# Arthur151/ROMP

Measured on NVIDIA H100. Metric: frames/sec 512x512 ROMP-HRNet32 (whole hot path), higher is better.
Workload: dtype bf16

## Files before the change

romp_b200/csrc/conv_block_tc.cu:

```cuda
#include "conv_tc.cuh"
#include "tc_device.cuh"

namespace b200romp {

namespace {

constexpr int kBlkThreads = 384;
constexpr int kRowB = 128;
constexpr int kHaloH = 20;
constexpr int kTapBytes = 64 * kRowB;
constexpr int kHalfTapBytes = 64 * 64;

template <bool FOLD>
struct BlkCfg {
  static constexpr int kWBytes = FOLD ? 3 * (kTapBytes + 2 * kHalfTapBytes) : 9 * kTapBytes;
  static constexpr int kTW = FOLD ? 16 : 8;
  static constexpr int kHaloW = kTW + 4;
  static constexpr int kN1 = FOLD ? 192 : 128;
  static constexpr int kN2 = 8 * kTW;
  static constexpr int kG2 = kN2 / 8;
  static constexpr int kMidRows = 2 * kN1;
  static constexpr int kStagePayload = kHaloH * kHaloW * kRowB;
  static constexpr int kStageBytes = ((kMidRows + 2 * kHaloW + 2) * kRowB + 1023) / 1024 * 1024;
  static constexpr int kMidBytes = kMidRows * kRowB;
// ... 22 lines not shown
}

__device__ __forceinline__ void consumers_bar_sync() { asm volatile("bar.sync 1, 256;" ::: "memory"); }

__device__ __forceinline__ void ldmatrix_x4_trans(uint32_t (&r)[4], uint32_t addr) {
  asm volatile("ldmatrix.sync.aligned.m8n8.x4.trans.shared.b16 {%0, %1, %2, %3}, [%4];"
               : "=r"(r[0]), "=r"(r[1]), "=r"(r[2]), "=r"(r[3])
               : "r"(addr));
}
__device__ __forceinline__ void stmatrix_x4_trans(uint32_t addr, const uint32_t (&r)[4]) {
  asm volatile("stmatrix.sync.aligned.m8n8.x4.trans.shared.b16 [%0], {%1, %2, %3, %4};" ::"r"(addr), "r"(r[0]), "r"(r[1]), "r"(r[2]),
               "r"(r[3])
               : "memory");
}
__device__ __forceinline__ void st_shared_zero16(uint32_t addr) {
  asm volatile("st.shared.v4.b32 [%0], {%1, %1, %1, %1};" ::"r"(addr), "r"(0) : "memory");
}
template <int N>
__device__ __forceinline__ void wgmma_bf16(float (&d)[N / 2], uint64_t a, uint64_t b, uint32_t scale_d) {
  if constexpr (N == 192) wgmma_n192_bf16(d, a, b, scale_d);
  else if constexpr (N == 128) wgmma_n128_bf16(d, a, b, scale_d);
  else wgmma_n64(d, a, b, scale_d, false);
}
template <typename T>
__device__ __forceinline__ T opaque(T v) {
  uint64_t u = (uint64_t)v;
  asm volatile("mov.b64 %0, %0;" : "+l"(u));
  return (T)u;
}
__device__ __forceinline__ uint32_t pack_bf16x2(float a, float b) {
  const __nv_bfloat162 v = __floats2bfloat162_rn(a, b);
  return *reinterpret_cast<const uint32_t*>(&v);
}

struct BlkThread {
  int g, w, l;
};
template <bool FOLD>
__device__ __forceinline__ int c2_oy0(int g) { return FOLD ? 0 : 8 * g; }
template <bool FOLD>
__device__ __forceinline__ int c2_ox0(int g) { return FOLD ? 8 * g : 0; }
struct BlkTile {
  int n, y0, x0;
  __device__ BlkTile(int tile, int tiles_x, int per_frame, int tw) {
    n = tile / per_frame;
    const int rem = tile % per_frame;
    y0 = (rem / tiles_x) * 16;
    x0 = (rem % tiles_x) * tw;
  }
};

template <bool FOLD>
__device__ __forceinline__ void conv1_issue(float (&acc)[BlkCfg<FOLD>::kN1 / 2], uint32_t a_base, uint32_t w1_base, int row0) {
  constexpr int kHaloW = BlkCfg<FOLD>::kHaloW, kN1 = BlkCfg<FOLD>::kN1;
#pragma unroll
  for (int j = 0; j < kN1 / 2; ++j) acc[j] = 0.f;
  uint32_t scale_d = 0;
  wgmma_fence();
#pragma unroll
  for (int tap = 0; tap < 9; ++tap) {
    const uint32_t b_tap = a_base + (uint32_t)((row0 + (tap / 3) * kHaloW + tap % 3) * kRowB);
#pragma unroll
    for (int k = 0; k < 4; ++k) {
      if (blk_skip<FOLD>(tap, k)) continue;
      wgmma_bf16<kN1>(acc, w_desc<FOLD>(w1_base, tap, k), make_smem_desc(b_tap + k * 32, 8 * kRowB, kSw128), scale_d);
      scale_d = 1;
    }
  }
  wgmma_commit();
}

template <bool FOLD>
__device__ __forceinline__ void load_residual(uint32_t (&rv)[BlkCfg<FOLD>::kG2][2], uint32_t a_base, const BlkThread& th) {
  constexpr int kHaloW = BlkCfg<FOLD>::kHaloW;
  const int q = th.l >> 3;
#pragma unroll
  for (int j0 = 0; j0 < BlkCfg<FOLD>::kG2; j0 += 2) {
    const int hr = (c2_oy0<FOLD>(th.g) + j0 + (q >> 1) + 2) * kHaloW + c2_ox0<FOLD>(th.g) + (th.l & 7) + 2;
    uint32_t r[4];
    ldmatrix_x4_trans(r, a_base + hr * kRowB + (((2 * th.w + (q & 1)) ^ (hr & 7)) << 4));
    rv[j0][0] = r[0]; rv[j0][1] = r[1]; rv[j0 + 1][0] = r[2]; rv[j0 + 1][1] = r[3];
  }
}

template <bool FOLD>
__device__ __forceinline__ void mid_epilogue(const float (&acc)[BlkCfg<FOLD>::kN1 / 2], uint32_t mid_base, const float* b1p, const ConvParams& p,
                                             const BlkTile& tl, const BlkThread& th, int row0) {
  constexpr int kHaloW = BlkCfg<FOLD>::kHaloW, kTW = BlkCfg<FOLD>::kTW, kN1 = BlkCfg<FOLD>::kN1;
  const float bias[2] = {__ldg(b1p + 16 * th.w + (th.l >> 2)), __ldg(b1p + 16 * th.w + (th.l >> 2) + 8)};
  const int q = th.l >> 3;
#pragma unroll
  for (int j0 = 0; j0 < kN1 / 8; j0 += 2) {
    uint32_t r[4];
#pragma unroll
    for (int i = 0; i < 4; ++i) {
      const int j = j0 + (i >> 1), e = i & 1;
      r[i] = pack_bf16x2(fmaxf(acc[4 * j + 2 * e] + bias[e], 0.f), fmaxf(acc[4 * j + 2 * e + 1] + bias[e], 0.f));
    }
    const int m = row0 + 8 * (j0 + (q >> 1)) + (th.l & 7);
    stmatrix_x4_trans(mid_base + m * kRowB + (((2 * th.w + (q & 1)) ^ (m & 7)) << 4), r);
  }
  if (tl.y0 > 0 && tl.x0 > 0 && tl.y0 + 16 < p.Hout && tl.x0 + kTW < p.Wout) return;
  __syncwarp();
  constexpr int kRingRow = kTW + 2, kRing = 2 * kRingRow + 2 * 18;
#pragma unroll 1
  for (int i = th.l; i < 2 * kRing; i += 32) {
    const int k = i >> 1;
    const int my = k < 2 * kRingRow ? (k < kRingRow ? 0 : 17) : (k - 2 * kRingRow) % 18;
    const int mx = k < 2 * kRingRow ? k % kRingRow : (k - 2 * kRingRow < 18 ? 0 : kTW + 1);
    const int m = my * kHaloW + mx;
    if (m >= row0 && m < row0 + kN1 && ((unsigned)(tl.y0 - 1 + my) >= (unsigned)p.Hout || (unsigned)(tl.x0 - 1 + mx) >= (unsigned)p.Wout))
      st_shared_zero16(mid_base + m * kRowB + (((2 * th.w + (i & 1)) ^ (m & 7)) << 4));
  }
}

template <bool FOLD>
__device__ __forceinline__ void conv2_issue(float (&acc2)[BlkCfg<FOLD>::kN2 / 2], uint32_t mid_base, uint32_t w2_base, int g) {
  constexpr int kHaloW = BlkCfg<FOLD>::kHaloW, kN2 = BlkCfg<FOLD>::kN2;
#pragma unroll
  for (int j = 0; j < kN2 / 2; ++j) acc2[j] = 0.f;
  uint32_t scale_d = 0;
  wgmma_fence();
#pragma unroll
  for (int tap = 0; tap < 9; ++tap) {
    const uint32_t b_tap = mid_base + (uint32_t)(((c2_oy0<FOLD>(g) + tap / 3) * kHaloW + c2_ox0<FOLD>(g) + tap % 3) * kRowB);
#pragma unroll
    for (int k = 0; k < 4; ++k) {
      if (blk_skip<FOLD>(tap, k)) continue;
      wgmma_bf16<kN2>(acc2, w_desc<FOLD>(w2_base, tap, k), make_smem_desc(b_tap + k * 32, kHaloW * kRowB, kSw128), scale_d);
      scale_d = 1;
    }
  }
  wgmma_commit();
}

template <bool FOLD>
__device__ __forceinline__ void out_epilogue(const float (&acc2)[BlkCfg<FOLD>::kN2 / 2], const uint32_t (&rv)[BlkCfg<FOLD>::kG2][2],
                                             const float* b2p, const ConvParams& p, const BlkTile& tl, const BlkThread& th) {
  __nv_bfloat16* out = reinterpret_cast<__nv_bfloat16*>(p.out);
  const int c = 16 * th.w + (th.l >> 2);
  const float bias[2] = {__ldg(b2p + c), __ldg(b2p + c + 8)};
  const int odd = (th.l >> 2) & 1;
  const int x = tl.x0 + c2_ox0<FOLD>(th.g) + 2 * (th.l & 3) + odd;
#pragma unroll
  for (int j = 0; j < BlkCfg<FOLD>::kG2; ++j) {
    uint16_t h[2][2];
#pragma unroll
    for (int e = 0; e < 2; ++e) {
      const float2 r = res_pair(rv[j][e]);
      const float a = (acc2[4 * j + 2 * e] + bias[e]) + r.x, b = (acc2[4 * j + 2 * e + 1] + bias[e]) + r.y;
      h[e][0] = __bfloat16_as_ushort(__float2bfloat16_rn(fmaxf(a, 0.f)));
      h[e][1] = __bfloat16_as_ushort(__float2bfloat16_rn(fmaxf(b, 0.f)));
    }
    const uint32_t send = odd ? (uint32_t)h[0][0] | ((uint32_t)h[1][0] << 16) : (uint32_t)h[0][1] | ((uint32_t)h[1][1] << 16);
    const uint32_t recv = __shfl_xor_sync(0xffffffffu, send, 4);
    const size_t pix = ((size_t)tl.n * p.Hout + tl.y0 + c2_oy0<FOLD>(th.g) + j) * p.Wout + x;
    uint32_t* o = reinterpret_cast<uint32_t*>(out + pix * p.out_C + p.out_c_off + (c & ~1));
#pragma unroll
    for (int e = 0; e < 2; ++e) {
      const uint32_t theirs = (recv >> (16 * e)) & 0xFFFFu;
      o[4 * e] = odd ? (theirs | ((uint32_t)h[e][1] << 16)) : ((uint32_t)h[e][0] | (theirs << 16));
    }
  }
}

}

template <bool FOLD>
__global__ void __launch_bounds__(kBlkThreads, 1)
conv_block_tc_kernel(const __grid_constant__ CUtensorMap tmap, const ConvParams p, const uint8_t* __restrict__ w1pack,
                     const uint8_t* __restrict__ w2pack, const float* __restrict__ bias1, int tiles_x, int tiles_y, int num_tiles) {
  using Cfg = BlkCfg<FOLD>;
  constexpr int kWBytes = Cfg::kWBytes, kStageBytes = Cfg::kStageBytes;
  extern __shared__ uint8_t smem_raw[];
  uint8_t* smem = reinterpret_cast<uint8_t*>((reinterpret_cast<uintptr_t>(smem_raw) + 1023) & ~(uintptr_t)1023);
  uint8_t* sW1 = smem;
  uint8_t* sW2 = smem + kWBytes;
  uint8_t* sA = smem + 2 * kWBytes;
  uint8_t* sMid = sA + kStageBytes;
  uint64_t* full = reinterpret_cast<uint64_t*>(sMid + Cfg::kMidBytes);
  uint64_t* empty = full + 1;
  uint64_t* w_full = full + 2;

  const int warp = threadIdx.x >> 5;
  if (threadIdx.x == 0) {
    mbar_init(full, 1);
    mbar_init(empty, 256);
    mbar_init(w_full, 1);
    fence_barrier_init();
  }
  __syncthreads();
  pdl_trigger();
  const int per_frame = tiles_x * tiles_y;

  if (warp == 0) {
    if (elect_one()) {
      mbar_arrive_expect_tx(w_full, 2 * kWBytes);
      for (int off = 0; off < kWBytes; off += kTapBytes) {
        bulk_copy_g2s(sW1 + off, w1pack + off, kTapBytes, w_full);
        bulk_copy_g2s(sW2 + off, w2pack + off, kTapBytes, w_full);
      }
      pdl_wait();
      const uint64_t pol = l2_policy_stream();
      uint32_t phase = 0;
      for (int tile = blockIdx.x; tile < num_tiles; tile += gridDim.x, phase ^= 1) {
        const BlkTile tl(tile, tiles_x, per_frame, Cfg::kTW);
        mbar_wait(empty, phase ^ 1);
        mbar_arrive_expect_tx(full, Cfg::kStagePayload);
        tma_load_4d(sA, &tmap, full, 0, tl.x0 - 2, tl.y0 - 2, tl.n, pol);
      }
    }
  } else if (warp >= 4) {
    const int t = threadIdx.x & 127;
    const BlkThread th{(warp >> 2) - 1, t >> 5, t & 31};
    pdl_wait();
    mbar_wait(w_full, 0);
    float acc[Cfg::kN1 / 2], acc2[Cfg::kN2 / 2];
    uint32_t rv[Cfg::kG2][2];
    const int row0 = th.g * Cfg::kN1;
    uint32_t phase = 0;
    for (int tile = blockIdx.x; tile < num_tiles; tile += gridDim.x, phase ^= 1) {
      const uint32_t w1_base = opaque(smem_u32(sW1)), w2_base = opaque(smem_u32(sW2)), a_base = opaque(smem_u32(sA)),
                     mid_base = opaque(smem_u32(sMid));
      const float* b1p = opaque(bias1);
      const float* b2p = opaque(p.bias);
      const BlkTile tl(tile, tiles_x, per_frame, Cfg::kTW);
      mbar_wait(full, phase);
      conv1_issue<FOLD>(acc, a_base, w1_base, row0);
      load_residual<FOLD>(rv, a_base, th);
      wgmma_wait<0>();
      mbar_arrive(empty);
      consumers_bar_sync();
      mid_epilogue<FOLD>(acc, mid_base, b1p, p, tl, th, row0);
      fence_proxy_async();
      consumers_bar_sync();
      conv2_issue<FOLD>(acc2, mid_base, w2_base, th.g);
      wgmma_wait<0>();
      out_epilogue<FOLD>(acc2, rv, b2p, p, tl, th);
    }
  }
}

bool tc_block_supported(const ConvParams& p, bool fold) {
  if (p.in_dtype != B200ROMP_BF16 || p.out_dtype != B200ROMP_BF16 || p.res_dtype != B200ROMP_BF16) return false;
  if (p.cin != 64 || p.cout != 64 || p.up != 1 || p.out_nchw || p.pow_channel >= 0 || p.input_norm || !p.relu) return false;
  if (p.Hin != p.Hout || p.Win != p.Wout || p.Hout % 16 != 0 || p.Wout % (fold ? BlkCfg<true>::kTW : BlkCfg<false>::kTW) != 0) return false;
  if (p.in_C % 8 != 0 || p.in_c_off % 8 != 0 || p.out_C % 8 != 0 || p.out_c_off % 8 != 0) return false;
  if (p.res != p.in || p.res_C != p.in_C || p.res_c_off != p.in_c_off || p.res_broadcast) return false;
  return (reinterpret_cast<uintptr_t>(p.in) & 15) == 0;
}

static int block_pack_weights(const float* w_oihw, bool fold, void** d_out, std::vector<void*>* allocs) {
  if (!fold) return tc_pack_weights(w_oihw, 64, 64, 9, 64, d_out, allocs, kRowB, 2);
  const std::vector<uint8_t> full = tc_pack_image(w_oihw, 64, 64, 9, 64, kRowB, 2);
  const std::vector<uint8_t> half = tc_pack_image(w_oihw, 64, 64, 9, 64, 64, 2);
  std::vector<uint8_t> img(BlkCfg<true>::kWBytes);
  for (int tap = 0; tap < 9; ++tap) {
    uint8_t* dst = img.data() + w_tap_off(true, tap);
    if (tap % 3 == 1) memcpy(dst, full.data() + (size_t)tap * kTapBytes, kTapBytes);
    else memcpy(dst, half.data() + (size_t)(2 * tap + (tap % 3 == 0 ? 1 : 0)) * kHalfTapBytes, kHalfTapBytes);
  }
  *d_out = upload(img.data(), img.size(), allocs);
  return *d_out ? B200ROMP_OK : B200ROMP_ECUDA;
}

int tc_block_prepare(const ConvParams& p, const float* w1_oihw, const float* b1, const float* w2_oihw, int sm_count,
                     TcConvPlan* plan, std::vector<void*>* allocs) {
  plan->kind = 60;
  plan->eb = 2;
  plan->cin = plan->cout = plan->nt = 64;
  plan->grid_x = sm_count;
  plan->grid_y = 1;
  plan->stages = 1;
  plan->smem_bytes = plan->fold ? BlkCfg<true>::kSmemBytes : BlkCfg<false>::kSmemBytes;
  int rc = block_pack_weights(w1_oihw, plan->fold, &plan->d_wpack, allocs);
  if (rc) return rc;
  rc = block_pack_weights(w2_oihw, plan->fold, &plan->d_wpack2, allocs);
  if (rc) return rc;
  plan->d_bias1 = static_cast<const float*>(upload(b1, 64 * sizeof(float), allocs));
  if (!plan->d_bias1) return B200ROMP_ECUDA;
  rc = tc_encode_nhwc_input(&plan->tmap_in, p, 2, 64, plan->fold ? BlkCfg<true>::kHaloW : BlkCfg<false>::kHaloW, kHaloH,
                            CU_TENSOR_MAP_SWIZZLE_128B, "conv_block_tc");
  if (rc) return rc;
  B2R_CUDA_OK(cudaFuncSetAttribute(conv_block_tc_kernel<false>, cudaFuncAttributeMaxDynamicSharedMemorySize, BlkCfg<false>::kSmemBytes));
  B2R_CUDA_OK(cudaFuncSetAttribute(conv_block_tc_kernel<true>, cudaFuncAttributeMaxDynamicSharedMemorySize, BlkCfg<true>::kSmemBytes));
  return B200ROMP_OK;
}

int tc_block_launch(const TcConvPlan& plan, const ConvParams& p, cudaStream_t stream) {
  const int tiles_x = p.Wout / (plan.fold ? BlkCfg<true>::kTW : BlkCfg<false>::kTW), tiles_y = p.Hout / 16;
  const int num_tiles = tiles_x * tiles_y * p.B;
  const dim3 grid(std::min(plan.grid_x, num_tiles));
  auto kern = plan.fold ? conv_block_tc_kernel<true> : conv_block_tc_kernel<false>;
  B2R_CUDA_OK(tc_launch(kern, grid, kBlkThreads, plan.smem_bytes, stream, plan.tmap_in, p, reinterpret_cast<const uint8_t*>(plan.d_wpack),
                        reinterpret_cast<const uint8_t*>(plan.d_wpack2), plan.d_bias1, tiles_x, tiles_y, num_tiles));
  return B200ROMP_OK;
}

}
```

romp_b200/csrc/conv_tc.cu:

```cuda
#include <mutex>

#include "conv_tc.cuh"
#include "tc_device.cuh"

namespace b200romp {

thread_local int g_tc_pdl_override = -1;

constexpr int kTcThreads = 384;
constexpr int kMaxRings = 2;

__host__ __device__ constexpr int s2_row_bytes(int cin, int eb) { return cin * eb >= 512 ? 64 : (cin * eb < 128 ? cin * eb : 128); }

__host__ __device__ constexpr int tc_num_rings(int stages) { return stages >= 4 ? kMaxRings : 1; }
__host__ __device__ constexpr int tc_ring_size(int stages, int ring) { return tc_num_rings(stages) == 1 ? stages : (stages + 1 - ring) / 2; }
__host__ __device__ constexpr int tc_ring_base(int stages, int ring) { return ring ? (stages + 1) / 2 : 0; }

template <int MODE, int CIN, int NT, int EB>
struct TcCfg {
  static constexpr bool S2 = MODE == 2;
  static constexpr int KS = MODE == 1 ? 1 : 3;
  static constexpr int TAPS = KS * KS;
  static constexpr int PAD = KS / 2;
  static constexpr int ROWB = S2 ? s2_row_bytes(CIN, EB) : tc_row_bytes(KS, CIN, EB);
  static constexpr int CW = ROWB / EB;
  static constexpr int KCH = CIN / CW;
  static constexpr int KSTEPS = ROWB / 32;
  static constexpr uint32_t LAYOUT = tc_layout(ROWB);
  static constexpr int HW_ = 8 + 2 * PAD;
  static constexpr int HH = 16 + 2 * PAD;
  __host__ __device__ static constexpr int BH(int i) { return i < 2 ? 17 : 16; }
  __host__ __device__ static constexpr int BW(int i) { return (i & 1) ? 8 : 9; }
  __host__ __device__ static constexpr int SUB_BYTES(int i) { return (BH(i) * BW(i) * ROWB + 1023) / 1024 * 1024; }
  __host__ __device__ static constexpr int SUB_OFF(int i) { return i == 0 ? 0 : SUB_OFF(i - 1) + SUB_BYTES(i - 1); }
  static constexpr int STAGE_PAYLOAD = S2 ? (17 * 9 + 17 * 8 + 16 * 9 + 16 * 8) * ROWB : HH * HW_ * ROWB;
  static constexpr int STAGE_BYTES = S2 ? SUB_OFF(3) + SUB_BYTES(3) : (STAGE_PAYLOAD + 1023) / 1024 * 1024;
  static constexpr int BTILE = NT * ROWB;
  static constexpr int B_BYTES = TAPS * KCH * BTILE;
  static constexpr bool FOLDABLE = MODE == 3 && CIN == 64 && NT == 64 && EB == 2;
};

template <int MODE, int CIN, int NT, int EB, bool GENERIC>
__global__ void __launch_bounds__(kTcThreads, 1)
conv_tc_kernel(const __grid_constant__ CUtensorMap tmap, const __grid_constant__ S2Maps s2maps, const ConvParams p,
               const uint8_t* __restrict__ wpack, int tiles_x, int tiles_y, int num_tiles, int stages, unsigned kmask) {
  using Cfg = TcCfg<MODE, CIN, NT, EB>;
  extern __shared__ uint8_t smem_raw[];
  uint8_t* smem = reinterpret_cast<uint8_t*>((reinterpret_cast<uintptr_t>(smem_raw) + 1023) & ~(uintptr_t)1023);
  uint8_t* sB = smem;
  uint8_t* sA = smem + Cfg::B_BYTES;
  uint64_t* full = reinterpret_cast<uint64_t*>(sA + (size_t)stages * Cfg::STAGE_BYTES);
  uint64_t* empty = full + stages;
  uint64_t* b_full = empty + stages;

  const int warp = threadIdx.x >> 5;
  if (threadIdx.x == 0) {
    for (int i = 0; i < stages; ++i) {
      mbar_init(&full[i], 1);
      mbar_init(&empty[i], 4);
    }
    mbar_init(b_full, 1);
    fence_barrier_init();
  }
  __syncthreads();
  pdl_trigger();
  const int per_frame = tiles_x * tiles_y;
  const int nrings = tc_num_rings(stages);

  if (warp == 0) {
    if (elect_one()) {
      mbar_arrive_expect_tx(b_full, Cfg::B_BYTES);
      const uint8_t* wsrc = wpack + (size_t)blockIdx.y * Cfg::B_BYTES;
      for (int i = 0; i < Cfg::TAPS * Cfg::KCH; ++i)
        bulk_copy_g2s(sB + (size_t)i * Cfg::BTILE, wsrc + (size_t)i * Cfg::BTILE, Cfg::BTILE, b_full);
      pdl_wait();
      const uint64_t pol = l2_policy_stream();
      int stage = 0, stage_other = 0;
      uint32_t phase = 0, phase_other = 0;
      int it = 0;
      for (int tile = blockIdx.x; tile < num_tiles; tile += gridDim.x, ++it) {
        const int n = tile / per_frame, rem = tile % per_frame;
        const int y0 = (rem / tiles_x) * 16, x0 = (rem % tiles_x) * 8;
        const int ring = nrings == 2 ? (it & 1) : 0, rbase = tc_ring_base(stages, ring), rsize = tc_ring_size(stages, ring);
        for (int c = 0; c < Cfg::KCH; ++c) {
          const int sidx = rbase + stage;
          mbar_wait(&empty[sidx], phase ^ 1);
          mbar_arrive_expect_tx(&full[sidx], Cfg::STAGE_PAYLOAD);
          uint8_t* dst = sA + (size_t)sidx * Cfg::STAGE_BYTES;
          if constexpr (Cfg::S2) {
#pragma unroll
            for (int i = 0; i < 4; ++i) {
              const int ph = i < 2 ? 1 : 0, pw = (i & 1) ? 0 : 1;
              tma_load_5d(dst + Cfg::SUB_OFF(i), &s2maps.m[i], &full[sidx], pw * p.in_C + p.in_c_off + c * Cfg::CW, x0 - pw, ph,
                          y0 - ph, n, pol);
            }
          } else {
            tma_load_4d(dst, &tmap, &full[sidx], c * Cfg::CW, x0 - Cfg::PAD, y0 - Cfg::PAD, n, pol);
          }
          if (++stage == rsize) { stage = 0; phase ^= 1; }
        }
        if (nrings == 2) { const int ts = stage; stage = stage_other; stage_other = ts; const uint32_t tp = phase; phase = phase_other; phase_other = tp; }
      }
    }
  } else if (warp >= 4 && (warp >> 2) <= nrings) {
    const int g = (warp >> 2) - 1, t = threadIdx.x & 127, wlane = threadIdx.x & 31;
    pdl_wait();
    mbar_wait(b_full, 0);
    const uint32_t b_base = smem_u32(sB);
    const int rbase = tc_ring_base(stages, g), rsize = tc_ring_size(stages, g);
    int stage = 0;
    uint32_t phase = 0;
    for (int tile = blockIdx.x + g * gridDim.x; tile < num_tiles; tile += nrings * gridDim.x) {
      const int n = tile / per_frame, rem = tile % per_frame;
      const int y0 = (rem / tiles_x) * 16, x0 = (rem % tiles_x) * 8;
      float acc[2][NT / 2];
#pragma unroll
      for (int h = 0; h < 2; ++h)
#pragma unroll
        for (int j = 0; j < NT / 2; ++j) acc[h][j] = 0.f;
      uint32_t scale_d = 0;
      int prev = -1;
      for (int c = 0; c < Cfg::KCH; ++c) {
        const int sidx = rbase + stage;
        mbar_wait(&full[sidx], phase);
        uint8_t* a_stage = sA + (size_t)sidx * Cfg::STAGE_BYTES;
        if constexpr (EB == 4) {
          tf32_round_smem(a_stage, Cfg::STAGE_BYTES, t, 128);
          fence_proxy_async();
          wg_bar_sync(1 + g);
        }
        const uint32_t a_base = smem_u32(a_stage);
        wgmma_fence();
#pragma unroll
        for (int tap = 0; tap < Cfg::TAPS; ++tap) {
          const int r = tap / Cfg::KS, s = tap % Cfg::KS;
          uint32_t a_tap, sbo;
          if constexpr (Cfg::S2) {
            const int sub = (r != 1 ? 0 : 2) + (s != 1 ? 0 : 1);
            const int bw = Cfg::BW(sub);
            a_tap = a_base + (uint32_t)(Cfg::SUB_OFF(sub) + ((r == 2 ? bw : 0) + (s == 2 ? 1 : 0)) * Cfg::ROWB);
            sbo = bw * Cfg::ROWB;
          } else {
            a_tap = a_base + (uint32_t)((r * Cfg::HW_ + s) * Cfg::ROWB);
            sbo = Cfg::HW_ * Cfg::ROWB;
          }
          const uint32_t b_tap = b_base + (uint32_t)((tap * Cfg::KCH + c) * Cfg::BTILE);
#pragma unroll
          for (int k = 0; k < Cfg::KSTEPS; ++k) {
            if (Cfg::FOLDABLE && !((kmask >> (tap * 2 + (k * 2) / Cfg::KSTEPS)) & 1u)) continue;
            const uint64_t bdesc = make_smem_desc(b_tap + k * 32, 8 * Cfg::ROWB, Cfg::LAYOUT);
            wgmma_any<NT, EB>(acc[0], make_smem_desc(a_tap + k * 32, sbo, Cfg::LAYOUT), bdesc, scale_d);
            wgmma_any<NT, EB>(acc[1], make_smem_desc(a_tap + 8 * sbo + k * 32, sbo, Cfg::LAYOUT), bdesc, scale_d);
            scale_d = 1;
          }
        }
        wgmma_commit();
        if (prev >= 0) {
          wgmma_wait<1>();
          if (wlane == 0) mbar_arrive(&empty[prev]);
        }
        prev = sidx;
        if (++stage == rsize) { stage = 0; phase ^= 1; }
      }
      wgmma_wait<0>();
      if (wlane == 0) mbar_arrive(&empty[prev]);
      wg_epilogue<NT, GENERIC ? kEpiGeneric : kEpiNhwc>(p, acc, p.bias, n, y0, x0, blockIdx.y * NT, t);
    }
  }
}

PFN_encodeTiled tc_get_encode() {
  static PFN_encodeTiled fn = nullptr;
  static std::once_flag once;
  std::call_once(once, [] {
    void* ptr = nullptr;
    cudaDriverEntryPointQueryResult qres;
    if (cudaGetDriverEntryPoint("cuTensorMapEncodeTiled", &ptr, cudaEnableDefault, &qres) == cudaSuccess &&
        qres == cudaDriverEntryPointSuccess)
      fn = reinterpret_cast<PFN_encodeTiled>(ptr);
  });
  return fn;
}

int tc_encode_tiled(CUtensorMap* map, CUtensorMapDataType dtype, int rank, const void* base, const cuuint64_t* dims,
                    const cuuint64_t* strides, const cuuint32_t* box, CUtensorMapSwizzle swizzle, const char* tag) {
  PFN_encodeTiled encode = tc_get_encode();
  if (!encode) {
    set_error("%s: cuTensorMapEncodeTiled is unavailable", tag);
    return B200ROMP_ECUDA;
  }
  const cuuint32_t estr[5] = {1, 1, 1, 1, 1};
  const CUresult cr = encode(map, dtype, rank, const_cast<void*>(base), dims, strides, box, estr, CU_TENSOR_MAP_INTERLEAVE_NONE,
                             swizzle, CU_TENSOR_MAP_L2_PROMOTION_L2_128B, CU_TENSOR_MAP_FLOAT_OOB_FILL_NONE);
  if (cr != CUDA_SUCCESS) {
    set_error("%s: cuTensorMapEncodeTiled failed with %d", tag, (int)cr);
    return B200ROMP_ECUDA;
  }
  return B200ROMP_OK;
}

int tc_encode_nhwc_input(CUtensorMap* map, const ConvParams& p, int eb, int box_c, int box_w, int box_h, CUtensorMapSwizzle swizzle,
                         const char* tag) {
  const cuuint64_t dims[4] = {(cuuint64_t)p.cin, (cuuint64_t)p.Win, (cuuint64_t)p.Hin, (cuuint64_t)p.B};
  const cuuint64_t strides[3] = {(cuuint64_t)p.in_C * eb, (cuuint64_t)p.Win * p.in_C * eb, (cuuint64_t)p.Hin * p.Win * p.in_C * eb};
  const cuuint32_t box[4] = {(cuuint32_t)box_c, (cuuint32_t)box_w, (cuuint32_t)box_h, 1};
  return tc_encode_tiled(map, eb == 2 ? CU_TENSOR_MAP_DATA_TYPE_BFLOAT16 : CU_TENSOR_MAP_DATA_TYPE_FLOAT32, 4,
                         static_cast<const uint8_t*>(p.in) + (size_t)p.in_c_off * eb, dims, strides, box, swizzle, tag);
}

float tc_round_tf32_host(float w) {
  uint32_t u;
  memcpy(&u, &w, 4);
  if ((u & 0x7F800000u) != 0x7F800000u) u = (u + 0x1000u) & ~0x1FFFu;
  float r;
  memcpy(&r, &u, 4);
  return r;
}

std::vector<uint8_t> tc_pack_image(const float* w_oihw, int cin, int cout, int taps, int nt, int rowb, int eb) {
  const int cw = rowb / eb, kch = cin / cw, ntiles = (cout + nt - 1) / nt, per16 = 16 / eb;
  std::vector<uint8_t> img((size_t)ntiles * taps * kch * nt * rowb, 0);
  for (int j = 0; j < ntiles; ++j)
    for (int t = 0; t < taps; ++t)
      for (int c = 0; c < kch; ++c) {
        uint8_t* tile = img.data() + (((size_t)j * taps + t) * kch + c) * nt * rowb;
        for (int n = 0; n < nt; ++n)
          for (int k = 0; k < cw; ++k) {
            const int co = j * nt + n, ci = c * cw + k;
            if (co >= cout) continue;
            const float w = w_oihw[((size_t)co * cin + ci) * taps + t];
            const int chunk16 = k / per16;
            const int phase = rowb == 128 ? (n & 7) : ((n >> 1) & 3);
            const size_t byte = (size_t)n * rowb + (size_t)((chunk16 ^ phase) * 16) + (k % per16) * eb;
            if (eb == 2) { const __nv_bfloat16 b = __float2bfloat16_rn(w); memcpy(tile + byte, &b, 2); }
            else { const float f = tc_round_tf32_host(w); memcpy(tile + byte, &f, 4); }
          }
      }
  return img;
}

int tc_pack_weights(const float* w_oihw, int cin, int cout, int taps, int nt, void** d_out, std::vector<void*>* allocs, int rowb, int eb) {
  const std::vector<uint8_t> img = tc_pack_image(w_oihw, cin, cout, taps, nt, rowb, eb);
  *d_out = upload(img.data(), img.size(), allocs);
  return *d_out ? B200ROMP_OK : B200ROMP_ECUDA;
}

std::string TcConvPlan::describe() const {
  char buf[128];
  snprintf(buf, sizeof(buf), " [tc%s k%d v%d nt%d grid %dx%d smem %d stages %d%s]", eb == 4 ? "-tf32" : "", kind / 10, kind % 10, nt, grid_x,
           grid_y, smem_bytes, stages, kmask != 0xFFFFFFFFu ? " pixel-pairs" : "");
  return buf;
}

static bool tc_s2_supported(const ConvParams& p) {
  if ((p.in_dtype != B200ROMP_BF16 && p.in_dtype != B200ROMP_F32) || p.input_norm || p.out_nchw || p.pow_channel >= 0) return false;
  const int eb = p.in_dtype == B200ROMP_F32 ? 4 : 2;
  if (eb == 4 && (p.out_dtype != B200ROMP_F32 || (p.res != nullptr && p.res_dtype != B200ROMP_F32))) return false;
  if (p.cin != 32 && p.cin != 64 && p.cin != 128 && p.cin != 256) return false;
  if (eb == 4 && p.cin == 256) return false;
  if (p.in_C % 8 != 0 || p.in_c_off % 8 != 0) return false;
  if (p.cout % 32 != 0 || p.Hin % 2 != 0 || p.Win % 2 != 0) return false;
  if (p.Hout % 16 != 0 || p.Wout % 8 != 0 || p.Hout * 2 != p.Hin || p.Wout * 2 != p.Win) return false;
  if (p.out_C % 8 != 0 || p.out_c_off % 8 != 0) return false;
  if (p.res != nullptr && (p.res_C % 8 != 0 || p.res_c_off % 8 != 0)) return false;
  if ((reinterpret_cast<uintptr_t>(p.in) & 15) != 0) return false;
  return true;
}

static bool tc_shape_supported(const ConvParams& p, int ksize, int stride) {
  if (stride == 2 && ksize == 3) return tc_s2_supported(p);
  if (stride != 1 || (ksize != 1 && ksize != 3)) return false;
  if ((p.in_dtype != B200ROMP_BF16 && p.in_dtype != B200ROMP_F32) || p.input_norm) return false;
  if (p.in_dtype == B200ROMP_F32 && (p.out_dtype != B200ROMP_F32 || (p.res != nullptr && p.res_dtype != B200ROMP_F32))) return false;
  if (p.cin != 32 && p.cin != 64 && p.cin != 128 && p.cin != 256) return false;
  if (p.Hout % 16 != 0 || p.Wout % 8 != 0) return false;
  if (p.in_C % 8 != 0 || p.in_c_off % 8 != 0) return false;
  if (p.out_nchw) {
    if (p.out_dtype != B200ROMP_F32 || p.up != 1 || p.res != nullptr) return false;
    return (reinterpret_cast<uintptr_t>(p.in) & 15) == 0;
  }
  if (p.pow_channel >= 0 || p.cout % 32 != 0) return false;
  if (p.out_C % 8 != 0 || p.out_c_off % 8 != 0) return false;
  if (p.res != nullptr && (p.res_C % 8 != 0 || p.res_c_off % 8 != 0)) return false;
  if ((reinterpret_cast<uintptr_t>(p.in) & 15) != 0) return false;
  return true;
}

static int tc_rowb(int ksize, int stride, int cin, int eb) { return stride == 2 ? s2_row_bytes(cin, eb) : tc_row_bytes(ksize, cin, eb); }

static bool tc_tile(const ConvParams& p, int ksize, int stride, TcConvPlan* plan) {
  const int eb = p.in_dtype == B200ROMP_F32 ? 4 : 2;
  const int rowb = tc_rowb(ksize, stride, p.cin, eb), kch = p.cin / (rowb / eb);
  const int budget = 227 * 1024 - 1024  - 1024 ;
  auto bbytes = [&](int n) { return ksize * ksize * kch * n * rowb; };
  int nt = (p.cout % 64 == 0) ? 64 : 32;
  int stage_bytes, stages;
  if (stride == 2) {
    auto sub_bytes = [&](int i) { return ((i < 2 ? 17 : 16) * ((i & 1) ? 8 : 9) * rowb + 1023) / 1024 * 1024; };
    stage_bytes = sub_bytes(0) + sub_bytes(1) + sub_bytes(2) + sub_bytes(3);
    if (nt == 64 && bbytes(64) + 2 * stage_bytes > budget && bbytes(32) + 2 * stage_bytes <= budget) nt = 32;
    if (nt == 64 && bbytes(64) + stage_bytes > budget) nt = 32;
    if (bbytes(nt) + stage_bytes > budget) return false;
    stages = std::min(4, (budget - bbytes(nt)) / stage_bytes);
  } else {
    const int hh = 16 + 2 * (ksize / 2), hw = 8 + 2 * (ksize / 2);
    stage_bytes = (hh * hw * rowb + 1023) / 1024 * 1024;
    if (bbytes(nt) + 3 * stage_bytes > budget && nt == 64) nt = 32;
    if (bbytes(nt) + 2 * stage_bytes > budget && nt == 32) nt = 16;
    if (bbytes(nt) + 2 * stage_bytes > budget) return false;
    stages = std::min((budget - bbytes(nt)) / stage_bytes, 8);
  }
  plan->kind = stride == 2 ? 32 : ksize * 10;
  plan->eb = eb;
  plan->cin = p.cin; plan->cout = p.cout; plan->nt = nt;
  plan->stages = stages;
  plan->smem_bytes = bbytes(nt) + stages * stage_bytes + 1024 + 1024;
  return true;
}

// ... 74 lines not shown
```

romp_b200/csrc/tc_device.cuh:

```cuda
#pragma once
#include <cuda.h>

#include <vector>

#include "conv_tc.cuh"

namespace b200romp {

__device__ __forceinline__ uint32_t smem_u32(const void* p) { return (uint32_t)__cvta_generic_to_shared(p); }

__device__ __forceinline__ void mbar_init(uint64_t* bar, uint32_t count) {
  asm volatile("mbarrier.init.shared::cta.b64 [%0], %1;" ::"r"(smem_u32(bar)), "r"(count) : "memory");
}
__device__ __forceinline__ void mbar_arrive_expect_tx(uint64_t* bar, uint32_t bytes) {
  asm volatile("mbarrier.arrive.expect_tx.shared::cta.b64 _, [%0], %1;" ::"r"(smem_u32(bar)), "r"(bytes) : "memory");
}
__device__ __forceinline__ void mbar_arrive(uint64_t* bar) {
  asm volatile("mbarrier.arrive.shared::cta.b64 _, [%0];" ::"r"(smem_u32(bar)) : "memory");
}
__device__ __forceinline__ bool mbar_try_wait(uint64_t* bar, uint32_t parity) {
  uint32_t ok;
  asm volatile(
      "{\n\t.reg .pred p;\n\t"
      "mbarrier.try_wait.parity.shared::cta.b64 p, [%1], %2;\n\t"
// ... 105 lines not shown
        "{\n\t.reg .pred p;\n\tsetp.ne.b32 p, %34, 0;\n\t"
        "wgmma.mma_async.sync.aligned.m64n64k8.f32.tf32.tf32 {%0, %1, %2, %3, %4, %5, %6, %7, %8, %9, %10, %11, %12, %13, %14, "
        "%15, %16, %17, %18, %19, %20, %21, %22, %23, %24, %25, %26, %27, %28, %29, %30, %31}, %32, %33, p, 1, 1;\n\t}"
        : B2R_WG_R8(0), B2R_WG_R8(8), B2R_WG_R8(16), B2R_WG_R8(24)
        : "l"(a), "l"(b), "r"(scale_d)
        : "memory");
}
__device__ __forceinline__ void wgmma_n128_bf16(float (&d)[64], uint64_t a, uint64_t b, uint32_t scale_d) {
  asm volatile(
      "{\n\t.reg .pred p;\n\tsetp.ne.b32 p, %66, 0;\n\t"
      "wgmma.mma_async.sync.aligned.m64n128k16.f32.bf16.bf16 {%0, %1, %2, %3, %4, %5, %6, %7, %8, %9, %10, %11, %12, %13, %14, "
      "%15, %16, %17, %18, %19, %20, %21, %22, %23, %24, %25, %26, %27, %28, %29, %30, %31, %32, %33, %34, %35, %36, %37, %38, "
      "%39, %40, %41, %42, %43, %44, %45, %46, %47, %48, %49, %50, %51, %52, %53, %54, %55, %56, %57, %58, %59, %60, %61, %62, "
      "%63}, %64, %65, p, 1, 1, 0, 0;\n\t}"
      : B2R_WG_R8(0), B2R_WG_R8(8), B2R_WG_R8(16), B2R_WG_R8(24), B2R_WG_R8(32), B2R_WG_R8(40), B2R_WG_R8(48), B2R_WG_R8(56)
      : "l"(a), "l"(b), "r"(scale_d)
      : "memory");
}
__device__ __forceinline__ void wgmma_n192_bf16(float (&d)[96], uint64_t a, uint64_t b, uint32_t scale_d) {
  asm volatile(
      "{\n\t.reg .pred p;\n\tsetp.ne.b32 p, %98, 0;\n\t"
      "wgmma.mma_async.sync.aligned.m64n192k16.f32.bf16.bf16 {%0, %1, %2, %3, %4, %5, %6, %7, %8, %9, %10, %11, %12, %13, %14, "
      "%15, %16, %17, %18, %19, %20, %21, %22, %23, %24, %25, %26, %27, %28, %29, %30, %31, %32, %33, %34, %35, %36, %37, %38, "
      "%39, %40, %41, %42, %43, %44, %45, %46, %47, %48, %49, %50, %51, %52, %53, %54, %55, %56, %57, %58, %59, %60, %61, %62, "
      "%63, %64, %65, %66, %67, %68, %69, %70, %71, %72, %73, %74, %75, %76, %77, %78, %79, %80, %81, %82, %83, %84, %85, %86, "
      "%87, %88, %89, %90, %91, %92, %93, %94, %95}, %96, %97, p, 1, 1, 0, 0;\n\t}"
      : B2R_WG_R8(0), B2R_WG_R8(8), B2R_WG_R8(16), B2R_WG_R8(24), B2R_WG_R8(32), B2R_WG_R8(40), B2R_WG_R8(48), B2R_WG_R8(56),
        B2R_WG_R8(64), B2R_WG_R8(72), B2R_WG_R8(80), B2R_WG_R8(88)
      : "l"(a), "l"(b), "r"(scale_d)
      : "memory");
}
#undef B2R_WG_R8
template <int NT, int EB>
__device__ __forceinline__ void wgmma_any(float (&d)[NT / 2], uint64_t a, uint64_t b, uint32_t scale_d) {
  if constexpr (NT == 64) wgmma_n64(d, a, b, scale_d, EB == 4);
  else if constexpr (NT == 32) wgmma_n32(d, a, b, scale_d, EB == 4);
  else wgmma_n16(d, a, b, scale_d, EB == 4);
}

constexpr uint32_t kSw128 = 1, kSw64 = 2;
__device__ __forceinline__ uint64_t make_smem_desc(uint32_t addr, uint32_t sbo_bytes, uint32_t layout) {
  return (uint64_t)((addr & 0x3FFFF) >> 4) | ((uint64_t)1 << 16) | ((uint64_t)(sbo_bytes >> 4) << 32) | ((uint64_t)layout << 62);
}
__host__ __device__ constexpr uint32_t tc_layout(int row_bytes) { return row_bytes == 128 ? kSw128 : kSw64; }

__host__ __device__ constexpr int tc_row_bytes(int ksize, int cin, int eb) {
  return (ksize == 3 && cin >= 128) ? 64 : (cin * eb < 128 ? cin * eb : 128);
}

__device__ __forceinline__ uint32_t tf32_rna(uint32_t x) {
  uint32_t y;
  asm("cvt.rna.tf32.f32 %0, %1;" : "=r"(y) : "r"(x));
  return y;
}
__device__ __forceinline__ void tf32_round_smem(uint8_t* base, int bytes, int t, int nthreads) {
  const uint32_t s0 = smem_u32(base);
  for (int off = t * 16; off < bytes; off += nthreads * 16) {
    uint32_t a, b, c, d;
    asm volatile("ld.shared.v4.b32 {%0, %1, %2, %3}, [%4];" : "=r"(a), "=r"(b), "=r"(c), "=r"(d) : "r"(s0 + off));
    a = tf32_rna(a); b = tf32_rna(b); c = tf32_rna(c); d = tf32_rna(d);
    asm volatile("st.shared.v4.b32 [%4], {%0, %1, %2, %3};" ::"r"(a), "r"(b), "r"(c), "r"(d), "r"(s0 + off) : "memory");
  }
}

__device__ __forceinline__ void wg_store2(const ConvParams& p, int n, int oy, int ox, int co, float v0, float v1) {
  if (p.out_nchw || p.pow_channel >= 0 || co + 2 > p.cout) {
    const float v[2] = {v0, v1};
    conv_epilogue_store<2>(p, n, oy, ox, co, v);
    return;
  }
  const int up = p.up, Hf = p.Hout * up, Wf = p.Wout * up;
  for (int dy = 0; dy < up; ++dy) {
    for (int dx = 0; dx < up; ++dx) {
      const int fy = oy * up + dy, fx = ox * up + dx;
      const size_t pix = ((size_t)n * Hf + fy) * Wf + fx;
      float a = v0, b = v1;
      if (p.res != nullptr) {
        const size_t ri = ((size_t)(p.res_broadcast ? 0 : n) * Hf + fy) * Wf + fx;
        const size_t idx = ri * p.res_C + p.res_c_off + co;
        if (p.res_dtype == B200ROMP_BF16) {
          const __nv_bfloat162 r = *reinterpret_cast<const __nv_bfloat162*>(reinterpret_cast<const __nv_bfloat16*>(p.res) + idx);
          a += __low2float(r); b += __high2float(r);
        } else {
          const float2 r = *reinterpret_cast<const float2*>(reinterpret_cast<const float*>(p.res) + idx);
          a += r.x; b += r.y;
        }
      }
      if (p.relu) { a = fmaxf(a, 0.f); b = fmaxf(b, 0.f); }
      const size_t oi = pix * p.out_C + p.out_c_off + co;
      if (p.out_dtype == B200ROMP_BF16)
        *reinterpret_cast<__nv_bfloat162*>(reinterpret_cast<__nv_bfloat16*>(p.out) + oi) = __floats2bfloat162_rn(a, b);
      else
        *reinterpret_cast<float2*>(reinterpret_cast<float*>(p.out) + oi) = make_float2(a, b);
    }
  }
}

__host__ __device__ __forceinline__ bool tc_nhwc_out(const ConvParams& p, int co_end) {
  return p.up == 1 && !p.out_nchw && p.pow_channel < 0 && co_end <= p.cout;
}

__device__ __forceinline__ float2 res_pair(uint32_t r) {
  const __nv_bfloat162 v = *reinterpret_cast<const __nv_bfloat162*>(&r);
  return make_float2(__low2float(v), __high2float(v));
}
__device__ __forceinline__ float2 res_pair(float2 r) { return r; }

template <int NT, typename RT, int ROWS = (NT / 8) * (int)sizeof(RT) <= 16 ? 4 : (NT / 8) * (int)sizeof(RT) <= 32 ? 2 : 1>
__device__ __forceinline__ void wg_epilogue_nhwc(const ConvParams& p, const float (&acc)[2][NT / 2], int n, int y0, int x0, int co0,
                                                 int w, int l, bool linear) {
  const int dpix = linear ? 8 : p.Wout;
  auto pix0 = [&](int frame) -> size_t {
    return linear ? ((size_t)frame * p.Hout + y0) * p.Wout + x0 + 16 * w + (l >> 2)
                  : ((size_t)frame * p.Hout + y0 + 2 * w) * p.Wout + x0 + (l >> 2);
  };
  const int c = co0 + 2 * (l & 3);
  const uint8_t* rbase = nullptr;
  int rstep = 0;
  if (p.res != nullptr) {
    rbase = reinterpret_cast<const uint8_t*>(p.res) + (pix0(p.res_broadcast ? 0 : n) * p.res_C + p.res_c_off + c) * (sizeof(RT) / 2);
    rstep = dpix * p.res_C * (int)(sizeof(RT) / 2);
  }
  const int ob = p.out_dtype == B200ROMP_BF16 ? 2 : 4;
  uint8_t* obase = reinterpret_cast<uint8_t*>(p.out) + (pix0(n) * p.out_C + p.out_c_off + c) * ob;
  const int ostep = dpix * p.out_C * ob;
#pragma unroll
  for (int q0 = 0; q0 < 4; q0 += ROWS) {
    RT rv[ROWS][NT / 8];
    if (p.res != nullptr) {
#pragma unroll
      for (int qq = 0; qq < ROWS; ++qq) {
        const int q = q0 + qq;
        const RT* r = reinterpret_cast<const RT*>(rbase + (8 * (q >> 1) + (q & 1)) * rstep);
#pragma unroll
        for (int j = 0; j < NT / 8; ++j) rv[qq][j] = r[4 * j];
      }
    }
#pragma unroll
    for (int qq = 0; qq < ROWS; ++qq) {
      const int q = q0 + qq, h = q >> 1, e = q & 1;
      uint8_t* o = obase + (8 * h + e) * ostep;
#pragma unroll
      for (int j = 0; j < NT / 8; ++j) {
        float a = acc[h][4 * j + 2 * e], b = acc[h][4 * j + 2 * e + 1];
        if (p.res != nullptr) { const float2 r = res_pair(rv[qq][j]); a += r.x; b += r.y; }
        if (p.relu) { a = fmaxf(a, 0.f); b = fmaxf(b, 0.f); }
        if (ob == 2) reinterpret_cast<__nv_bfloat162*>(o)[4 * j] = __floats2bfloat162_rn(a, b);
        else reinterpret_cast<float2*>(o)[4 * j] = make_float2(a, b);
      }
    }
  }
}

constexpr int kEpiNhwc = 0, kEpiGeneric = 1, kEpiAny = 2;
template <int NT, int PATH = kEpiAny>
__device__ __forceinline__ void wg_epilogue(const ConvParams& p, float (&acc)[2][NT / 2], const float* __restrict__ bias, int n,
                                            int y0, int x0, int co0, int wg_thread, bool linear = false) {
  const int w = wg_thread >> 5, l = wg_thread & 31;
  if (PATH == kEpiNhwc || (PATH == kEpiAny && tc_nhwc_out(p, co0 + NT))) {
#pragma unroll
    for (int j = 0; j < NT / 8; ++j) {
      const int c = co0 + 8 * j + 2 * (l & 3);
      const float b0 = __ldg(bias + c), b1 = __ldg(bias + c + 1);
#pragma unroll
      for (int h = 0; h < 2; ++h) {
        acc[h][4 * j] += b0; acc[h][4 * j + 1] += b1; acc[h][4 * j + 2] += b0; acc[h][4 * j + 3] += b1;
      }
    }
    if (p.res != nullptr && p.res_dtype == B200ROMP_F32) wg_epilogue_nhwc<NT, float2>(p, acc, n, y0, x0, co0, w, l, linear);
    else wg_epilogue_nhwc<NT, uint32_t>(p, acc, n, y0, x0, co0, w, l, linear);
    return;
  }
  if constexpr (PATH != kEpiNhwc) {
#pragma unroll
    for (int h = 0; h < 2; ++h) {
#pragma unroll
      for (int j = 0; j < NT / 8; ++j) {
        const int c = co0 + 8 * j + 2 * (l & 3);
        const float b0 = __ldg(bias + c), b1 = __ldg(bias + c + 1);
#pragma unroll
        for (int e = 0; e < 2; ++e) {
          const int m = 64 * h + 16 * w + (l >> 2) + 8 * e;
          wg_store2(p, n, linear ? y0 : y0 + (m >> 3), linear ? x0 + m : x0 + (m & 7), c, acc[h][4 * j + 2 * e] + b0,
                    acc[h][4 * j + 2 * e + 1] + b1);
        }
      }
    }
  }
}

template <typename... KArgs, typename... Args>
static inline cudaError_t tc_launch(void (*kern)(KArgs...), dim3 grid, int threads, int smem_bytes, cudaStream_t stream, Args&&... args) {
  static const bool pdl_default = [] { const char* e = getenv("B200ROMP_NO_PDL"); return !(e && e[0] == '1'); }();
  const bool pdl = pdl_default && g_tc_pdl_override != 0;
  cudaLaunchConfig_t cfg = {};
  cfg.gridDim = grid;
  cfg.blockDim = dim3(threads);
  cfg.dynamicSmemBytes = (size_t)smem_bytes;
  cfg.stream = stream;
  cudaLaunchAttribute at[1];
  at[0].id = cudaLaunchAttributeProgrammaticStreamSerialization;
  at[0].val.programmaticStreamSerializationAllowed = 1;
  cfg.attrs = at;
  cfg.numAttrs = pdl ? 1 : 0;
  return cudaLaunchKernelEx(&cfg, kern, static_cast<KArgs>(args)...);
}

typedef CUresult (*PFN_encodeTiled)(CUtensorMap*, CUtensorMapDataType, cuuint32_t, void*, const cuuint64_t*, const cuuint64_t*,
                                    const cuuint32_t*, const cuuint32_t*, CUtensorMapInterleave, CUtensorMapSwizzle,
                                    CUtensorMapL2promotion, CUtensorMapFloatOOBfill);
PFN_encodeTiled tc_get_encode();
int tc_encode_tiled(CUtensorMap* map, CUtensorMapDataType dtype, int rank, const void* base, const cuuint64_t* dims,
                    const cuuint64_t* strides, const cuuint32_t* box, CUtensorMapSwizzle swizzle, const char* tag);
int tc_encode_nhwc_input(CUtensorMap* map, const ConvParams& p, int eb, int box_c, int box_w, int box_h, CUtensorMapSwizzle swizzle,
                         const char* tag);
std::vector<uint8_t> tc_pack_image(const float* w_oihw, int cin, int cout, int taps, int nt, int rowb, int eb);
int tc_pack_weights(const float* w_oihw, int cin, int cout, int taps, int nt, void** d_out, std::vector<void*>* allocs, int rowb, int eb);
float tc_round_tf32_host(float w);

}
```

Before: 3596.

## Swap wgmma operands so weights form M and pixels form a single N128 instruction

For 3x3 and stride-2 bf16 convs with 64 output channels, the generic kernel now issues one wgmma with weights as the A operand and the 128-pixel tile as N=128, replacing two M64xN64 instructions per k-step. Output accumulators come out channel-major, so a new epilogue swaps pairs across lanes with shuffles, adds bias and residual, and writes NHWC bf16 or fp32. The bf16 residual is loaded before waiting on wgmma to hide its latency. The fused block kernel's epilogue is also rewritten to use the shared pair-swap helper and byte_perm packing. The aim is fewer wgmma issues and better B-operand reuse, at the cost of extra shuffle work and register pressure in the epilogue.

```diff
diff --git a/romp_b200/csrc/conv_block_tc.cu b/romp_b200/csrc/conv_block_tc.cu
--- a/romp_b200/csrc/conv_block_tc.cu
+++ b/romp_b200/csrc/conv_block_tc.cu
@@ -198,15 +198,12 @@
       h[e][0] = __bfloat16_as_ushort(__float2bfloat16_rn(fmaxf(a, 0.f)));
       h[e][1] = __bfloat16_as_ushort(__float2bfloat16_rn(fmaxf(b, 0.f)));
     }
-    const uint32_t send = odd ? (uint32_t)h[0][0] | ((uint32_t)h[1][0] << 16) : (uint32_t)h[0][1] | ((uint32_t)h[1][1] << 16);
-    const uint32_t recv = __shfl_xor_sync(0xffffffffu, send, 4);
+    uint32_t lo = (uint32_t)h[0][0] | ((uint32_t)h[1][0] << 16), hi = (uint32_t)h[0][1] | ((uint32_t)h[1][1] << 16);
+    cm_pair_swap(lo, hi, odd);
     const size_t pix = ((size_t)tl.n * p.Hout + tl.y0 + c2_oy0<FOLD>(th.g) + j) * p.Wout + x;
     uint32_t* o = reinterpret_cast<uint32_t*>(out + pix * p.out_C + p.out_c_off + (c & ~1));
-#pragma unroll
-    for (int e = 0; e < 2; ++e) {
-      const uint32_t theirs = (recv >> (16 * e)) & 0xFFFFu;
-      o[4 * e] = odd ? (theirs | ((uint32_t)h[e][1] << 16)) : ((uint32_t)h[e][0] | (theirs << 16));
-    }
+    o[0] = __byte_perm(lo, hi, 0x5410);
+    o[4] = __byte_perm(lo, hi, 0x7632);
   }
 }
 
diff --git a/romp_b200/csrc/conv_tc.cu b/romp_b200/csrc/conv_tc.cu
--- a/romp_b200/csrc/conv_tc.cu
+++ b/romp_b200/csrc/conv_tc.cu
@@ -45,6 +45,7 @@
 conv_tc_kernel(const __grid_constant__ CUtensorMap tmap, const __grid_constant__ S2Maps s2maps, const ConvParams p,
                const uint8_t* __restrict__ wpack, int tiles_x, int tiles_y, int num_tiles, int stages, unsigned kmask) {
   using Cfg = TcCfg<MODE, CIN, NT, EB>;
+  constexpr bool kSwap = MODE != 1 && NT == 64 && EB == 2 && !GENERIC;
   extern __shared__ uint8_t smem_raw[];
   uint8_t* smem = reinterpret_cast<uint8_t*>((reinterpret_cast<uintptr_t>(smem_raw) + 1023) & ~(uintptr_t)1023);
   uint8_t* sB = smem;
@@ -134,23 +135,27 @@
 #pragma unroll
         for (int tap = 0; tap < Cfg::TAPS; ++tap) {
           const int r = tap / Cfg::KS, s = tap % Cfg::KS;
-          uint32_t a_tap, sbo;
+          uint32_t px_tap, sbo;
           if constexpr (Cfg::S2) {
             const int sub = (r != 1 ? 0 : 2) + (s != 1 ? 0 : 1);
             const int bw = Cfg::BW(sub);
-            a_tap = a_base + (uint32_t)(Cfg::SUB_OFF(sub) + ((r == 2 ? bw : 0) + (s == 2 ? 1 : 0)) * Cfg::ROWB);
+            px_tap = a_base + (uint32_t)(Cfg::SUB_OFF(sub) + ((r == 2 ? bw : 0) + (s == 2 ? 1 : 0)) * Cfg::ROWB);
             sbo = bw * Cfg::ROWB;
           } else {
-            a_tap = a_base + (uint32_t)((r * Cfg::HW_ + s) * Cfg::ROWB);
+            px_tap = a_base + (uint32_t)((r * Cfg::HW_ + s) * Cfg::ROWB);
             sbo = Cfg::HW_ * Cfg::ROWB;
           }
-          const uint32_t b_tap = b_base + (uint32_t)((tap * Cfg::KCH + c) * Cfg::BTILE);
+          const uint32_t w_tap = b_base + (uint32_t)((tap * Cfg::KCH + c) * Cfg::BTILE);
 #pragma unroll
           for (int k = 0; k < Cfg::KSTEPS; ++k) {
             if (Cfg::FOLDABLE && !((kmask >> (tap * 2 + (k * 2) / Cfg::KSTEPS)) & 1u)) continue;
-            const uint64_t bdesc = make_smem_desc(b_tap + k * 32, 8 * Cfg::ROWB, Cfg::LAYOUT);
-            wgmma_any<NT, EB>(acc[0], make_smem_desc(a_tap + k * 32, sbo, Cfg::LAYOUT), bdesc, scale_d);
-            wgmma_any<NT, EB>(acc[1], make_smem_desc(a_tap + 8 * sbo + k * 32, sbo, Cfg::LAYOUT), bdesc, scale_d);
+            const uint64_t wdesc = make_smem_desc(w_tap + k * 32, 8 * Cfg::ROWB, Cfg::LAYOUT);
+            if constexpr (kSwap) {
+              wgmma_n128_bf16(reinterpret_cast<float(&)[64]>(acc), wdesc, make_smem_desc(px_tap + k * 32, sbo, Cfg::LAYOUT), scale_d);
+            } else {
+              wgmma_any<NT, EB>(acc[0], make_smem_desc(px_tap + k * 32, sbo, Cfg::LAYOUT), wdesc, scale_d);
+              wgmma_any<NT, EB>(acc[1], make_smem_desc(px_tap + 8 * sbo + k * 32, sbo, Cfg::LAYOUT), wdesc, scale_d);
+            }
             scale_d = 1;
           }
         }
@@ -162,9 +167,26 @@
         prev = sidx;
         if (++stage == rsize) { stage = 0; phase ^= 1; }
       }
+      const bool res_bf16 = kSwap && p.res != nullptr && p.res_dtype == B200ROMP_BF16;
+      uint32_t rv[16][2];
+      if (res_bf16) cm_load_residual<uint32_t, 16>(rv, p, n, y0, x0, blockIdx.y * NT, t, 0);
       wgmma_wait<0>();
       if (wlane == 0) mbar_arrive(&empty[prev]);
-      wg_epilogue<NT, GENERIC ? kEpiGeneric : kEpiNhwc>(p, acc, p.bias, n, y0, x0, blockIdx.y * NT, t);
+      if constexpr (kSwap) {
+        const float(&acc_cm)[64] = reinterpret_cast<const float(&)[64]>(acc);
+        if (p.res == nullptr || res_bf16) {
+          cm_store_rows<uint32_t, 16>(p, acc_cm, p.bias, rv, n, y0, x0, blockIdx.y * NT, t, 0);
+        } else {
+#pragma unroll
+          for (int j0 = 0; j0 < 16; j0 += 4) {
+            float2 rf[4][2];
+            cm_load_residual<float2, 4>(rf, p, n, y0, x0, blockIdx.y * NT, t, j0);
+            cm_store_rows<float2, 4>(p, acc_cm, p.bias, rf, n, y0, x0, blockIdx.y * NT, t, j0);
+          }
+        }
+      } else {
+        wg_epilogue<NT, GENERIC ? kEpiGeneric : kEpiNhwc>(p, acc, p.bias, n, y0, x0, blockIdx.y * NT, t);
+      }
     }
   }
 }
diff --git a/romp_b200/csrc/tc_device.cuh b/romp_b200/csrc/tc_device.cuh
--- a/romp_b200/csrc/tc_device.cuh
+++ b/romp_b200/csrc/tc_device.cuh
@@ -281,6 +281,55 @@
   }
 }
 
+template <typename T>
+__device__ __forceinline__ void cm_pair_swap(T& lo, T& hi, bool odd) {
+  const T recv = __shfl_xor_sync(0xffffffffu, odd ? lo : hi, 4);
+  if (odd) lo = recv;
+  else hi = recv;
+}
+
+__device__ __forceinline__ size_t cm_pixel(const ConvParams& p, int frame, int y0, int x0, int l, int j) {
+  return ((size_t)frame * p.Hout + y0 + j) * p.Wout + x0 + 2 * (l & 3) + ((l >> 2) & 1);
+}
+__device__ __forceinline__ int cm_channel(int co0, int wg_thread) { return co0 + 16 * (wg_thread >> 5) + ((wg_thread & 31) >> 2); }
+
+template <typename RT, int ROWS>
+__device__ __forceinline__ void cm_load_residual(RT (&rv)[ROWS][2], const ConvParams& p, int n, int y0, int x0, int co0, int wg_thread,
+                                                 int j0) {
+  const int c = cm_channel(co0, wg_thread);
+  const RT* r0 = reinterpret_cast<const RT*>(p.res) + (cm_pixel(p, p.res_broadcast ? 0 : n, y0, x0, wg_thread & 31, j0) * p.res_C + p.res_c_off + (c & ~1)) / 2;
+  const size_t rstep = (size_t)p.Wout * p.res_C / 2;
+#pragma unroll
+  for (int jj = 0; jj < ROWS; ++jj) {
+    rv[jj][0] = r0[jj * rstep];
+    rv[jj][1] = r0[jj * rstep + 4];
+  }
+}
+
+template <typename RT, int ROWS>
+__device__ __forceinline__ void cm_store_rows(const ConvParams& p, const float (&acc)[64], const float* __restrict__ bias, const RT (&rv)[ROWS][2],
+                                              int n, int y0, int x0, int co0, int wg_thread, int j0) {
+  const int l = wg_thread & 31, odd = (l >> 2) & 1, c = cm_channel(co0, wg_thread);
+  const float b[2] = {__ldg(bias + c), __ldg(bias + c + 8)};
+  const int ob = p.out_dtype == B200ROMP_BF16 ? 2 : 4;
+  uint8_t* obase = reinterpret_cast<uint8_t*>(p.out) + (cm_pixel(p, n, y0, x0, l, j0) * p.out_C + p.out_c_off + (c & ~1)) * ob;
+  const size_t ostep = (size_t)p.Wout * p.out_C * ob;
+#pragma unroll
+  for (int jj = 0; jj < ROWS; ++jj) {
+    const int j = j0 + jj;
+    uint8_t* o = obase + jj * ostep;
+#pragma unroll
+    for (int e = 0; e < 2; ++e) {
+      float lo = acc[4 * j + 2 * e] + b[e], hi = acc[4 * j + 2 * e + 1] + b[e];
+      cm_pair_swap(lo, hi, odd);
+      if (p.res != nullptr) { const float2 r = res_pair(rv[jj][e]); lo += r.x; hi += r.y; }
+      if (p.relu) { lo = fmaxf(lo, 0.f); hi = fmaxf(hi, 0.f); }
+      if (ob == 2) reinterpret_cast<__nv_bfloat162*>(o)[4 * e] = __floats2bfloat162_rn(lo, hi);
+      else reinterpret_cast<float2*>(o)[4 * e] = make_float2(lo, hi);
+    }
+  }
+}
+
 constexpr int kEpiNhwc = 0, kEpiGeneric = 1, kEpiAny = 2;
 template <int NT, int PATH = kEpiAny>
 __device__ __forceinline__ void wg_epilogue(const ConvParams& p, float (&acc)[2][NT / 2], const float* __restrict__ bias, int n,
```

Measured after the change: 3674, median of 6. 1.02x the previous value.
